# tjhladish/AbcSmc

Measured on AMD Instinct MI355X. Metric: particles/sec per SMC generation (PLS+weight+resample), 1/2/4/8 GPU, higher is better.
Workload: dtype f64 (inputs, model, distances, proposals, results; pair sums of the weight stage: fp64 operands as three f16 limbs on the matrix pipe + f32 v_exp_f32, weights <= 5e-7 rel of the fp64 oracle, largest seen 3.1e-7); 1 GPU; configs[2]: synthetic 1M particles x 16 params x 32 metrics, PLS 8 components, full generation; particles_per_gpu=1000000, particles_total=1000000, metrics=32, params=16, pls_components=8, pred_prior_size=100000, prev_pred_prior_size=100000, next_set_size=1000000, noise=MULTIVARIATE, ncomp_chosen=8, pls_component_rule=wilcoxon, parallelism=row-sharded x1, launcher=single GPU

## Files before the change

### abcsmc_amd/csrc/weights.hip

```cpp
#include <stdlib.h>

#include "abc_internal.h"
#include <hip/hip_ext.h>

namespace {

__device__ __forceinline__ double wave_sum(double v) {
#pragma unroll
    for (int o = 32; o >= 1; o >>= 1) v += __shfl_xor(v, o, 64);
    return v;
}

__device__ __forceinline__ double block_sum_256(double v, double* sm ) {
    v = wave_sum(v);
    __syncthreads();
    if ((threadIdx.x & 63) == 0) sm[threadIdx.x >> 6] = v;
    __syncthreads();
    return (sm[0] + sm[1]) + (sm[2] + sm[3]);
}

__global__ __launch_bounds__(256) void k_gather_rows(const double* __restrict__ Y, size_t n_local, size_t ldy,
                                                     int P, const unsigned long long* __restrict__ idx, size_t K,
                                                     unsigned long long idx_base, double* __restrict__ theta,
                                                     size_t ldt, const int* __restrict__ sel_fail, int* __restrict__ sel_fail_pin,
// ... 487 lines not shown
    double s = 0.0;
    for (int q = 0; q < n; q++) {
        const size_t j = sl[q];
        s += ks_pair_term<PP>(ai, ha, b + j * PP, hb[j]);
    }
    fix_j[i] = s;
}
template <int PP>
__global__ __launch_bounds__(256) void k_kde_fixups(const double* __restrict__ a, size_t kn, const double* __restrict__ b, size_t Kp,
                                                    const double* __restrict__ hb, const WConst* __restrict__ wc,
                                                    const unsigned char* __restrict__ far_flag, const unsigned* __restrict__ list,
                                                    unsigned nat, unsigned rb, unsigned slices, double* __restrict__ fix_i,
                                                    double* __restrict__ fix_j, const double* __restrict__ theta_raw, size_t K, size_t k0,
                                                    const double* __restrict__ prev_raw, double* __restrict__ part) {
    if (blockIdx.x < nat + rb) { far_body<PP>(blockIdx.x, a, kn, b, Kp, hb, wc, far_flag, list, nat, fix_i, fix_j); return; }
    const unsigned bid = blockIdx.x - (nat + rb);
    kde_body<PP>(bid % rb, bid / rb, slices, a, kn, b, Kp, hb, wc, theta_raw, K, k0, prev_raw, part, 1);
}

constexpr signed char KS_LA[KS_NP] = {0, 0, 1, 1, 2, 3};
constexpr signed char KS_LB[KS_NP] = {0, 1, 0, 1, 3, 2};
__device__ __forceinline__ float ks_max3(float a, float b, float c) {
    float r;
    asm volatile("v_max3_f32 %0, %1, %2, %3" : "=v"(r) : "v"(a), "v"(b), "v"(c));
    return r;
}
struct KsRef { float p0, p1, p2, p3; };
template <int V> __host__ __device__ constexpr int kz_nch() { return V > KS_TOPN ? V - KS_TOPN : V > KS_FOLD ? V - KS_FOLD : V; }
template <int V> __host__ __device__ constexpr bool kz_fold() { return V > KS_FOLD && V < KS_TOPN; }
template <int V> __host__ __device__ constexpr bool kz_topn() { return V > KS_TOPN; }
template <int V> __host__ __device__ constexpr int kz_nexact() { return V > KS_FOLD ? kz_nch<V>() : 1 + V; }
template <int NCH>
__host__ __device__ constexpr int kz_nsteps() { return kz_fold<NCH>() ? 1 + 6 * kz_nch<NCH>() : kz_topn<NCH>() ? 2 + 6 * kz_nch<NCH>() : 3 + 6 * NCH; }
template <int NCH, int S, typename AT>
__device__ __forceinline__ void kz_mfma(const AT A, const uint4* B, const uint4 (&NB)[2], const uint4& BN, f32x16& Z) {
    const f32x16 Z0 = {0.f, 0.f, 0.f, 0.f, 0.f, 0.f, 0.f, 0.f, 0.f, 0.f, 0.f, 0.f, 0.f, 0.f, 0.f, 0.f};
    if constexpr (kz_fold<NCH>()) {
        constexpr int C = kz_nch<NCH>();
        if constexpr (S == 0) {
            Z = __builtin_amdgcn_mfma_f32_32x32x16_f16(__builtin_bit_cast(f16x8, A[0]), __builtin_bit_cast(f16x8, B[0]), Z0, 0, 0, 0);
        } else if constexpr (S < C) {
            Z = __builtin_amdgcn_mfma_f32_32x32x16_f16(__builtin_bit_cast(f16x8, A[S * KS_NL]), __builtin_bit_cast(f16x8, B[S * KS_NL]), Z, 0, 0, 0);
        } else if constexpr (S == C) {
            Z = __builtin_amdgcn_mfma_f32_32x32x16_bf16(__builtin_bit_cast(bf16x8, NB[0]), __builtin_bit_cast(bf16x8, BN), Z, 0, 0, 0);
        } else {
            constexpr int q = S - (C + 1), c = q / 5, l = 1 + q % 5;
            Z = __builtin_amdgcn_mfma_f32_32x32x16_f16(__builtin_bit_cast(f16x8, A[c * KS_NL + KS_LA[l]]),
                                                       __builtin_bit_cast(f16x8, B[c * KS_NL + KS_LB[l]]), Z, 0, 0, 0);
        }
    } else if constexpr (kz_topn<NCH>()) {
        constexpr int C = kz_nch<NCH>();
        if constexpr (S == 0) {
            if (__builtin_amdgcn_readfirstlane(A[C * KS_NL + 1].y) == 0u) {
                Z = __builtin_amdgcn_mfma_f32_32x32x16_bf16(__builtin_bit_cast(bf16x8, A[C * KS_NL]), __builtin_bit_cast(bf16x8, NB[0]), Z0, 0, 0, 0);
                Z = __builtin_amdgcn_mfma_f32_32x32x16_f16(__builtin_bit_cast(f16x8, A[0]), __builtin_bit_cast(f16x8, B[0]), Z, 0, 0, 0);
            } else {
                Z = __builtin_amdgcn_mfma_f32_32x32x16_f16(__builtin_bit_cast(f16x8, A[0]), __builtin_bit_cast(f16x8, B[0]), Z0, 0, 0, 0);
            }
        } else if constexpr (S < C) {
            Z = __builtin_amdgcn_mfma_f32_32x32x16_f16(__builtin_bit_cast(f16x8, A[S * KS_NL]), __builtin_bit_cast(f16x8, B[S * KS_NL]), Z, 0, 0, 0);
        } else if constexpr (S == C) {
            Z = __builtin_amdgcn_mfma_f32_32x32x16_bf16(__builtin_bit_cast(bf16x8, A[C * KS_NL]), __builtin_bit_cast(bf16x8, BN), Z, 0, 0, 0);
        } else if constexpr (S == C + 1) {
            Z = __builtin_amdgcn_mfma_f32_32x32x16_bf16(__builtin_bit_cast(bf16x8, A[C * KS_NL]), __builtin_bit_cast(bf16x8, NB[1]), Z, 0, 0, 0);
        } else {
            constexpr int q = S - (C + 2), c = q / 5, l = 1 + q % 5;
            Z = __builtin_amdgcn_mfma_f32_32x32x16_f16(__builtin_bit_cast(f16x8, A[c * KS_NL + KS_LA[l]]),
                                                       __builtin_bit_cast(f16x8, B[c * KS_NL + KS_LB[l]]), Z, 0, 0, 0);
        }
    } else if constexpr (S == 0) {
        Z = __builtin_amdgcn_mfma_f32_32x32x16_bf16(__builtin_bit_cast(bf16x8, A[NCH * KS_NL]), __builtin_bit_cast(bf16x8, NB[0]), Z0, 0, 0, 0);
    } else if constexpr (S <= NCH) {
        constexpr int c = S - 1;
        Z = __builtin_amdgcn_mfma_f32_32x32x16_f16(__builtin_bit_cast(f16x8, A[c * KS_NL]), __builtin_bit_cast(f16x8, B[c * KS_NL]), Z, 0, 0, 0);
    } else if constexpr (S == NCH + 1) {
        Z = __builtin_amdgcn_mfma_f32_32x32x16_bf16(__builtin_bit_cast(bf16x8, A[NCH * KS_NL]), __builtin_bit_cast(bf16x8, BN), Z, 0, 0, 0);
    } else if constexpr (S == NCH + 2) {
        Z = __builtin_amdgcn_mfma_f32_32x32x16_bf16(__builtin_bit_cast(bf16x8, A[NCH * KS_NL]), __builtin_bit_cast(bf16x8, NB[1]), Z, 0, 0, 0);
    } else {
        constexpr int q = S - (NCH + 3), c = q / 5, l = 1 + q % 5;
        Z = __builtin_amdgcn_mfma_f32_32x32x16_f16(__builtin_bit_cast(f16x8, A[c * KS_NL + KS_LA[l]]),
                                                   __builtin_bit_cast(f16x8, B[c * KS_NL + KS_LB[l]]), Z, 0, 0, 0);
    }
}
template <int NCH, int S0, int S1, typename AT>
__device__ __forceinline__ void kz_mfma_range(const AT A, const uint4* B, const uint4 (&NB)[2], const uint4& BN, f32x16& Z) {
    if constexpr (S0 < S1) {
        kz_mfma<NCH, S0>(A, B, NB, BN, Z);
        kz_mfma_range<NCH, S0 + 1, S1>(A, B, NB, BN, Z);
    }
}
template <int V, typename AT>
__device__ __forceinline__ void kz_reference(const f32x16& Z, const AT A, const uint4& NB0, unsigned lane, int& n, uint4& BN) {
    const float f0 = __builtin_canonicalizef(Z[0]);
    __builtin_amdgcn_sched_barrier(0);
    const float m0 = ks_max3(f0, Z[1], Z[2]), m1 = ks_max3(Z[3], Z[4], Z[5]), m2 = ks_max3(Z[6], Z[7], Z[8]),
                m3 = ks_max3(Z[9], Z[10], Z[11]), m4 = ks_max3(Z[12], Z[13], Z[14]);
    const float ma = ks_max3(m0, m1, m2), mb = ks_max3(m3, m4, Z[15]);
    float m = ks_max3(ma, mb, mb);
    if constexpr (kz_topn<V>()) {
        const uint4 ti = A[kz_nch<V>() * KS_NL + 1];
        m -= __uint_as_float(ti.x);
        BN.x = NB0.x & ti.y;
        BN.y = NB0.y & ti.y;
    }
    const float nf = __builtin_floorf(m);
    n = (int)nf;
    typedef __attribute__((ext_vector_type(2))) float f32x2_;
    typedef __attribute__((ext_vector_type(2))) __bf16 bf16x2_;
    const bf16x2_ h1 = __builtin_convertvector((f32x2_){nf, 0.f}, bf16x2_);
    const float p1 = __uint_as_float(__builtin_bit_cast(unsigned, h1) << 16);
    const bf16x2_ pk = __builtin_convertvector((f32x2_){nf, nf - p1}, bf16x2_);
    (void)lane;
    BN.w = __builtin_bit_cast(unsigned, pk);
}
template <int NCH, int R, typename AT>
__device__ __forceinline__ void kz_slots(const AT An, const uint4* Bn, const uint4 (&NB)[2], f32x16& Zn, int& nn, unsigned lane,
                                         const f32x16& Zc, int nc, int hsub, double& s, KsRef& q, uint4& BN) {
    if constexpr (R < 8) {
        constexpr int NS = kz_nsteps<NCH>(), NA = kz_nexact<NCH>();
        if constexpr (R == 0) kz_mfma_range<NCH, 0, NA>(An, Bn, NB, BN, Zn);
        if constexpr (R == 3) {
            kz_reference<NCH>(Zn, An, NB[0], lane, nn, BN);
        }
        if constexpr (R >= 3 && R < 7) {
            constexpr int r = R - 3, M = NS - NA;
            constexpr int s0 = NA + (r * M) / 4, s1 = NA + ((r + 1) * M) / 4;
            if constexpr (r > 0) asm volatile("" : "+v"(Zn));
            kz_mfma_range<NCH, s0, s1>(An, Bn, NB, BN, Zn);
        }
#pragma unroll
        for (int g = 0; g < 2; g++) {
            const int i = R * 2 + g;
            const float e = __builtin_amdgcn_exp2f(Zc[i]);
            float& p = (i & 3) == 0 ? q.p0 : (i & 3) == 1 ? q.p1 : (i & 3) == 2 ? q.p2 : q.p3;
            if (i < 4) p = e; else p += e;
        }
        if constexpr (R == 7) {
            float t = q.p0 + q.p1;
            asm volatile("" : "+v"(t));
            t += q.p2 + q.p3;
            s += ldexp((double)t, nc - hsub);
            asm volatile("" : "+v"(s));
        } else {
            asm volatile("" : "+v"(q.p0), "+v"(q.p1), "+v"(q.p2), "+v"(q.p3));
        }
        __builtin_amdgcn_sched_barrier(0);
        kz_slots<NCH, R + 1>(An, Bn, NB, Zn, nn, lane, Zc, nc, hsub, s, q, BN);
    }
}

template <int NCH, int RO, int R, typename AT>
__device__ __forceinline__ void kz_fine(const AT An, const uint4* Bn, const uint4 (&NB)[2], f32x16& Zn, int& nn, unsigned lane,
                                        const f32x16& Zc, int nc, int hsub, double& s, KsRef& q, uint4& BN) {
    if constexpr (R < 16) {
        constexpr int NS = kz_nsteps<NCH>(), NA = kz_nexact<NCH>(), R0 = NA + RO, M = NS - NA, L = 16 - R0;
        if constexpr (R < NA) kz_mfma_range<NCH, R, R + 1>(An, Bn, NB, BN, Zn);
        if constexpr (R == R0) kz_reference<NCH>(Zn, An, NB[0], lane, nn, BN);
        if constexpr (R >= R0) {
            constexpr int r = R - R0;
            constexpr int s0 = NA + (r * M) / L, s1 = NA + ((r + 1) * M) / L;
            if constexpr (r > 0) asm volatile("" : "+v"(Zn));
            kz_mfma_range<NCH, s0, s1>(An, Bn, NB, BN, Zn);
        }
        {
            const float e = __builtin_amdgcn_exp2f(Zc[R]);
            float& p = (R & 3) == 0 ? q.p0 : (R & 3) == 1 ? q.p1 : (R & 3) == 2 ? q.p2 : q.p3;
            if (R < 4) p = e; else p += e;
        }
        if constexpr (R == 15) {
            float t = q.p0 + q.p1;
            asm volatile("" : "+v"(t));
            t += q.p2 + q.p3;
            s += ldexp((double)t, nc - hsub);
            asm volatile("" : "+v"(s));
        } else {
            asm volatile("" : "+v"(q.p0), "+v"(q.p1), "+v"(q.p2), "+v"(q.p3));
        }
        __builtin_amdgcn_sched_barrier(0);
        kz_fine<NCH, RO, R + 1>(An, Bn, NB, Zn, nn, lane, Zc, nc, hsub, s, q, BN);
    }
}
template <int NCH, int FINE, typename AT>
__device__ __forceinline__ void kz_step(const AT An, const uint4* Bn, const uint4 (&NB)[2], f32x16& Zn, int& nn, unsigned lane,
                                        const f32x16& Zc, int nc, int hsub, double& s, KsRef& q, uint4& BN) {
    if constexpr (FINE > 0) kz_fine<NCH, FINE, 0>(An, Bn, NB, Zn, nn, lane, Zc, nc, hsub, s, q, BN);
    else kz_slots<NCH, 0>(An, Bn, NB, Zn, nn, lane, Zc, nc, hsub, s, q, BN);
}

template <int NCH, int WPS, bool PING = (NCH >= 4), int FINE = 0>
__global__ __launch_bounds__(256, WPS) void k_kde_split(const uint4* __restrict__ at, size_t kn,
                                                      const uint4* __restrict__ bt, unsigned nbt,
                                                      const WConst* __restrict__ wc, const int* __restrict__ ha_int,
                                                      double* __restrict__ part, const uint2* __restrict__ tmin ) {
    if (!ks_split_on(wc)) return;
    constexpr int OPA = kz_nch<NCH>() * KS_NL, OPB = OPA + (kz_fold<NCH>() ? 0 : 1);
    constexpr int OPT = kz_topn<NCH>() ? 1 : 0;
    const unsigned lane = threadIdx.x & 63, wv = threadIdx.x >> 6;
    const size_t it0 = ((size_t)blockIdx.x * 4 + wv) * 2;
    const unsigned slices = gridDim.y, sl = blockIdx.y;
    const unsigned t0 = __builtin_amdgcn_readfirstlane((unsigned)((size_t)nbt * sl / slices));
    const unsigned t1 = __builtin_amdgcn_readfirstlane((unsigned)((size_t)nbt * (sl + 1) / slices));
    uint4 B0[OPA], B1[OPA];
#pragma unroll
    for (int q = 0; q < OPA; q++) {
        B0[q] = at[((it0 + 0) * OPA + q) * 64 + lane];
        B1[q] = at[((it0 + 1) * OPA + q) * 64 + lane];
    }
    uint4 NB[2];
    NB[0] = (lane < 32) ? make_uint4(KS_MONE | (KS_MONE << 16), KS_MONE, 0u, 0u) : make_uint4(0u, 0u, 0u, 0u);
    NB[1] = (lane < 32) ? make_uint4(0u, KS_MONE << 16, KS_MONE | (KS_MONE << 16), 0u) : make_uint4(0u, 0u, 0u, 0u);
    if constexpr (kz_fold<NCH>()) {
        const bool mine = (lane < 32) == (((lane & 31u) & 4u) == 0u);
        NB[0] = make_uint4(0u, 0u, 0u, mine ? (KS_MONE | (KS_MONE << 16)) : 0u);
    }
    const int hs0 = ha_int[(it0 + 0) * 32 + (lane & 31)], hs1 = ha_int[(it0 + 1) * 32 + (lane & 31)];
    double acc0 = 0.0, acc1 = 0.0;
    if (t0 < t1) {
        uint4 A[OPB + OPT];
#pragma unroll
        for (int q = 0; q < OPB; q++) A[q] = bt[((size_t)t0 * OPB + q) * 64 + lane];
        if constexpr (OPT) { const uint2 ti = tmin[t0]; A[OPB] = make_uint4(ti.x, ti.y, 0u, 0u); }
        f32x16 Z0, Z1;
        int n0 = 0, n1 = 0;
        uint4 BN = make_uint4(0u, 0u, 0u, 0u);
        {
            constexpr int NA = kz_nexact<NCH>();
            kz_mfma_range<NCH, 0, NA>(A, B0, NB, BN, Z0);
            kz_reference<NCH>(Z0, A, NB[0], lane, n0, BN);
            kz_mfma_range<NCH, NA, kz_nsteps<NCH>()>(A, B0, NB, BN, Z0);
        }
        if constexpr (!PING) {
        for (unsigned t = t0; t < t1; t++) {
            uint4 An[OPB + OPT];
            const unsigned tn = (t + 1 < t1) ? t + 1 : t;
#pragma unroll
            for (int q = 0; q < OPB; q++) An[q] = bt[((size_t)tn * OPB + q) * 64 + lane];
            if constexpr (OPT) { const uint2 ti = tmin[tn]; An[OPB] = make_uint4(ti.x, ti.y, 0u, 0u); }
            __builtin_amdgcn_sched_barrier(0);
            KsRef q;
            kz_step<NCH, FINE>(A, B1, NB, Z1, n1, lane, Z0, n0, hs0, acc0, q, BN);
            kz_step<NCH, FINE>(An, B0, NB, Z0, n0, lane, Z1, n1, hs1, acc1, q, BN);
#pragma unroll
            for (int q2 = 0; q2 < OPB; q2++) A[q2] = An[q2];
            if constexpr (OPT) { A[OPB].x = An[OPB].x; A[OPB].y = An[OPB].y; }
        }
        } else {
        uint4 An[OPB + OPT];
        for (unsigned t = t0; t < t1; t += 2) {
            {
                const unsigned tn = (t + 1 < t1) ? t + 1 : t;
#pragma unroll
                for (int q = 0; q < OPB; q++) An[q] = bt[((size_t)tn * OPB + q) * 64 + lane];
                if constexpr (OPT) { const uint2 ti = tmin[tn]; An[OPB] = make_uint4(ti.x, ti.y, 0u, 0u); }
            }
            __builtin_amdgcn_sched_barrier(0);
            KsRef q;
            kz_step<NCH, FINE>(A, B1, NB, Z1, n1, lane, Z0, n0, hs0, acc0, q, BN);
            kz_step<NCH, FINE>(An, B0, NB, Z0, n0, lane, Z1, n1, hs1, acc1, q, BN);
            if (t + 1 >= t1) break;
            {
                const unsigned tn = (t + 2 < t1) ? t + 2 : t + 1;
#pragma unroll
                for (int q2 = 0; q2 < OPB; q2++) A[q2] = bt[((size_t)tn * OPB + q2) * 64 + lane];
                if constexpr (OPT) { const uint2 ti = tmin[tn]; A[OPB] = make_uint4(ti.x, ti.y, 0u, 0u); }
            }
            __builtin_amdgcn_sched_barrier(0);
            kz_step<NCH, FINE>(An, B1, NB, Z1, n1, lane, Z0, n0, hs0, acc0, q, BN);
            kz_step<NCH, FINE>(A, B0, NB, Z0, n0, lane, Z1, n1, hs1, acc1, q, BN);
        }
        }
    }
    {
        const double v0 = acc0 + __shfl_xor(acc0, 32, 64);
        const double v1 = acc1 + __shfl_xor(acc1, 32, 64);
        const size_t i0 = (it0 + 0) * 32 + (lane & 31), i1 = (it0 + 1) * 32 + (lane & 31);
        if (lane < 32 && i0 < kn) part[(size_t)sl * kn + i0] = v0;
        if (lane < 32 && i1 < kn) part[(size_t)sl * kn + i1] = v1;
    }
}

template <int INFO>
struct KsLdsOps {
    const uint4* p;
    uint4 info;
    __device__ __forceinline__ const uint4& operator[](int i) const { return (INFO >= 0 && i == INFO) ? info : p[i * 64]; }
};
#ifndef KDE_LDS_F4
#define KDE_LDS_F4 0
#endif
#ifndef KDE_LDS_W3
#define KDE_LDS_W3 3
#endif
template <int NCH, int WPS, int FINE>
__global__ __launch_bounds__(256, WPS) void k_kde_split_lds(const uint4* __restrict__ at, size_t kn,
                                                          const uint4* __restrict__ bt, unsigned nbt,
                                                          const WConst* __restrict__ wc, const int* __restrict__ ha_int,
                                                          double* __restrict__ part, const uint2* __restrict__ tmin) {
    if (!ks_split_on(wc)) return;
    constexpr int OPA = kz_nch<NCH>() * KS_NL, OPB = OPA + (kz_fold<NCH>() ? 0 : 1);
    constexpr int OPT = kz_topn<NCH>() ? 1 : 0;
    constexpr int TILE = OPB * 64, NR = OPA / 4;
    __shared__ uint4 sA[2 * TILE];
    const unsigned lane = threadIdx.x & 63, wv = threadIdx.x >> 6;
    const size_t it0 = ((size_t)blockIdx.x * 4 + wv) * 2;
    const unsigned slices = gridDim.y, sl = blockIdx.y;
    const unsigned t0 = __builtin_amdgcn_readfirstlane((unsigned)((size_t)nbt * sl / slices));
    const unsigned t1 = __builtin_amdgcn_readfirstlane((unsigned)((size_t)nbt * (sl + 1) / slices));
    uint4 B0[OPA], B1[OPA];
#pragma unroll
    for (int q = 0; q < OPA; q++) {
        B0[q] = at[((it0 + 0) * OPA + q) * 64 + lane];
        B1[q] = at[((it0 + 1) * OPA + q) * 64 + lane];
    }
    uint4 NB[2];
    NB[0] = (lane < 32) ? make_uint4(KS_MONE | (KS_MONE << 16), KS_MONE, 0u, 0u) : make_uint4(0u, 0u, 0u, 0u);
    NB[1] = (lane < 32) ? make_uint4(0u, KS_MONE << 16, KS_MONE | (KS_MONE << 16), 0u) : make_uint4(0u, 0u, 0u, 0u);
    if constexpr (kz_fold<NCH>()) {
        const bool mine = (lane < 32) == (((lane & 31u) & 4u) == 0u);
        NB[0] = make_uint4(0u, 0u, 0u, mine ? (KS_MONE | (KS_MONE << 16)) : 0u);
    }
    const int hs0 = ha_int[(it0 + 0) * 32 + (lane & 31)], hs1 = ha_int[(it0 + 1) * 32 + (lane & 31)];
    double acc0 = 0.0, acc1 = 0.0;
    if (t0 < t1) {
        uint4 r[NR], r4 = make_uint4(0u, 0u, 0u, 0u);
        static_assert(OPA * 64 == NR * 256, "a tile's limb operands are whole rounds of the work-group");
#define KZ_TILE_FETCH(T)                                                                                            \
        {                                                                                                           \
            const uint4* src = bt + (size_t)(T) * (OPB * 64) + threadIdx.x;                                         \
            _Pragma("unroll") for (int j = 0; j < NR; j++) r[j] = src[256 * j];                                     \
            if constexpr (OPB > OPA) { if (threadIdx.x < 64) r4 = src[256 * NR]; }                                  \
        }
#define KZ_TILE_STORE(BUF)                                                                                          \
        {                                                                                                           \
            uint4* dst = sA + (BUF) * TILE + threadIdx.x;                                                           \
            _Pragma("unroll") for (int j = 0; j < NR; j++) dst[256 * j] = r[j];                                     \
            if constexpr (OPB > OPA) { if (threadIdx.x < 64) dst[256 * NR] = r4; }                                  \
        }
        KZ_TILE_FETCH(t0)
        KZ_TILE_STORE(0)
        __syncthreads();
        f32x16 Z0, Z1;
        int n0 = 0, n1 = 0;
        uint4 BN = make_uint4(0u, 0u, 0u, 0u);
        unsigned cur = 0;
        {
            constexpr int NA = kz_nexact<NCH>();
            KsLdsOps<OPT ? OPB : -1> A{sA + lane, make_uint4(0u, 0u, 0u, 0u)};
            if constexpr (OPT) { const uint2 ti = tmin[t0]; A.info = make_uint4(ti.x, ti.y, 0u, 0u); }
            kz_mfma_range<NCH, 0, NA>(A, B0, NB, BN, Z0);
            kz_reference<NCH>(Z0, A, NB[0], lane, n0, BN);
            kz_mfma_range<NCH, NA, kz_nsteps<NCH>()>(A, B0, NB, BN, Z0);
        }
        for (unsigned t = t0; t < t1; t++) {
            const unsigned tn = (t + 1 < t1) ? t + 1 : t;
            KZ_TILE_FETCH(tn)
            __builtin_amdgcn_sched_barrier(0);
            KsLdsOps<OPT ? OPB : -1> A{sA + cur * TILE + lane, make_uint4(0u, 0u, 0u, 0u)}, An{sA + (cur ^ 1u) * TILE + lane, make_uint4(0u, 0u, 0u, 0u)};
            if constexpr (OPT) {
                const uint2 ti = tmin[t], tj = tmin[tn];
                A.info = make_uint4(ti.x, ti.y, 0u, 0u);
                An.info = make_uint4(tj.x, tj.y, 0u, 0u);
            }
            KsRef q;
            kz_step<NCH, FINE>(A, B1, NB, Z1, n1, lane, Z0, n0, hs0, acc0, q, BN);
            KZ_TILE_STORE(cur ^ 1u)
            __syncthreads();
            kz_step<NCH, FINE>(An, B0, NB, Z0, n0, lane, Z1, n1, hs1, acc1, q, BN);
            cur ^= 1u;
        }
#undef KZ_TILE_FETCH
#undef KZ_TILE_STORE
    }
    {
        const double v0 = acc0 + __shfl_xor(acc0, 32, 64);
        const double v1 = acc1 + __shfl_xor(acc1, 32, 64);
        const size_t i0 = (it0 + 0) * 32 + (lane & 31), i1 = (it0 + 1) * 32 + (lane & 31);
        if (lane < 32 && i0 < kn) part[(size_t)sl * kn + i0] = v0;
        if (lane < 32 && i1 < kn) part[(size_t)sl * kn + i1] = v1;
    }
}

__device__ __forceinline__ double gaussian_pdf(double x, double sigma) {
    const double u = x / fabs(sigma);
    return (1.0 / (sqrt(2.0 * M_PI) * fabs(sigma))) * exp(-u * u / 2.0);
}

__device__ __forceinline__ double prior_likelihood(const abc_prior& pr, double v) {
    if (pr.kind == ABC_PRIOR_GAUSS) return gaussian_pdf(v - pr.a, pr.b);
    if (pr.kind == ABC_PRIOR_UNIF_INT)
        return ((v == round(v)) && (pr.a <= v) && (v <= pr.b)) ? 1.0 / (pr.b - pr.a + 1.0) : 0.0;
    return ((pr.a <= v) && (v <= pr.b)) ? 1.0 / (pr.b - pr.a) : 0.0;
}

constexpr unsigned SQ_INLINE_MAX = 4096;
__device__ __forceinline__ double sumsq_total(const double* __restrict__ sq_part, unsigned nparts, double* sm ) {
    double t = 0.0;
    for (unsigned j = threadIdx.x; j < nparts; j += 256) t += sq_part[j];
    return block_sum_256(t, sm);
}
__global__ __launch_bounds__(256) void k_sumsq_total(const double* __restrict__ sq_part, unsigned nparts, double* __restrict__ sq_total) {
    __shared__ double sm[4];
    const double t = sumsq_total(sq_part, nparts, sm);
    if (threadIdx.x == 0) *sq_total = t;
// ... 163 lines not shown
    for (int i = i0; i < i0 + per && i < total; i++) sum += bh[i];
    unsigned inc = sum;
#pragma unroll
    for (int o = 1; o < 64; o <<= 1) { const unsigned u = __shfl_up(inc, o, 64); if (lane >= o) inc += u; }
    if (lane == 63) wsum[wave] = inc;
    __syncthreads();
    unsigned run = inc - sum;
    for (int w = 0; w < wave; w++) run += wsum[w];
    for (int i = i0; i < i0 + per && i < total; i++) { const unsigned v = bh[i]; bh[i] = run; run += v; }
}
__global__ __launch_bounds__(256) void k_wq_rank(const double* __restrict__ hbk, size_t Kp, const WConst* __restrict__ wc,
                                                 const unsigned* __restrict__ bh, int nb, unsigned* __restrict__ rank) {
    __shared__ unsigned whist[4][256];
    __shared__ volatile unsigned woff[4][256];
    const int t = threadIdx.x, lane = t & 63, wave = t >> 6;
#pragma unroll
    for (int w = 0; w < 4; w++) whist[w][t] = 0;
    __syncthreads();
    const double lo = ks_okey_inv(wc->hb_lo), hi = ks_okey_inv(wc->hb_hi);
    const size_t seg = (size_t)blockIdx.x * WQ_CHUNK + (size_t)wave * (WQ_CHUNK / 4);
    unsigned q[WQ_ITEMS];
#pragma unroll
    for (int j = 0; j < WQ_ITEMS; j++) {
        const size_t i = seg + (size_t)j * 64 + lane;
        q[j] = (i < Kp) ? ks_qbin(hbk[i], lo, hi) : 0u;
        if (i < Kp) atomicAdd(&whist[wave][q[j]], 1u);
    }
    __syncthreads();
    {
        unsigned run = bh[(size_t)t * nb + blockIdx.x];
#pragma unroll
        for (int w = 0; w < 4; w++) { woff[w][t] = run; run += whist[w][t]; }
    }
    __syncthreads();
    const unsigned long long lt_mask = (lane == 0) ? 0ull : (~0ull >> (64 - lane));
#pragma unroll
    for (int j = 0; j < WQ_ITEMS; j++) {
        const size_t i = seg + (size_t)j * 64 + lane;
        const bool valid = i < Kp;
        const unsigned d = q[j];
        unsigned long long peers = __ballot(valid);
#pragma unroll
        for (int b = 0; b < 8; b++) {
            const unsigned long long m = __ballot((d >> b) & 1u);
            peers &= ((d >> b) & 1u) ? m : ~m;
        }
        if (valid) rank[i] = woff[wave][d] + (unsigned)__popcll(peers & lt_mask);
        __builtin_amdgcn_wave_barrier();
        if (valid && (peers & lt_mask) == 0) woff[wave][d] += (unsigned)__popcll(peers);
        __builtin_amdgcn_wave_barrier();
    }
}
constexpr float KS_TOPN_SPREAD = 0.75f;
__global__ __launch_bounds__(256) void k_tile_tmin(const float* __restrict__ topf, size_t ntiles, uint2* __restrict__ tinfo) {
    const size_t t = (size_t)blockIdx.x * 256 + threadIdx.x;
    if (t >= ntiles) return;
    float mn = 3.0e38f, mx = -3.0e38f;
    for (int j = 0; j < 32; j++) {
        const float v = topf[t * 32 + j];
        if (v < (float)KS_HB_ZERO) { mn = v < mn ? v : mn; mx = v > mx ? v : mx; }
    }
    if (mx < mn) { mn = (float)KS_HB_ZERO; mx = mn; }
    const bool wide = !(mx - mn <= KS_TOPN_SPREAD);
    tinfo[t] = wide ? make_uint2(0u, 0u) : make_uint2(__float_as_uint(mn), 0xffffffffu);
}
static double ks_topn_min_pairs() {
    const char* e = abc_diag_env("ABC_KDE_TOPN_MIN_PAIRS");
    const double minp = e ? atof(e) : 4.0e9;
    return minp;
}

using WrowsFn = decltype(&k_wrows<1>);
struct WrowsEntry { WrowsFn fn; int div; };
static const WrowsEntry WROWS[4] = {{k_wrows<1>, 32}, {k_wrows<2>, 16}, {k_wrows<4, 3>, 8}, {k_wrows<4>, 8}};

using SplitFn = decltype(&k_kde_split<1, 3, true, 1>);
static const SplitFn KDE_SPLIT[3][4] = {
    {k_kde_split<1, 3, true, 1>,
     k_kde_split<2, 2>,
     k_kde_split_lds<3, KDE_LDS_W3, KDE_LDS_F4>,
     k_kde_split_lds<4, 2, KDE_LDS_F4>},
    {k_kde_split<KS_FOLD + 1, 3, true, 1>,
     k_kde_split<KS_FOLD + 2, 2, false, 0>,
     k_kde_split_lds<KS_FOLD + 3, KDE_LDS_W3, KDE_LDS_F4>,
     k_kde_split_lds<KS_FOLD + 4, 2, KDE_LDS_F4>},
    {k_kde_split<KS_TOPN + 1, 3, true, 1>,
     k_kde_split<KS_TOPN + 2, 2, false, 0>,
     k_kde_split_lds<KS_TOPN + 3, KDE_LDS_W3, KDE_LDS_F4>,
     k_kde_split_lds<KS_TOPN + 4, 2, KDE_LDS_F4>},
};

using KdeFn = decltype(&k_kde<2>);
using EpanFn = decltype(&k_epan<2>);
using FixupsFn = decltype(&k_kde_fixups<8>);
static const KdeFn KDE_FP64[7] = {nullptr, k_kde<2>, k_kde<4>, k_kde<8>, k_kde<16>, k_kde<32>, k_kde<64>};
static const EpanFn KDE_EPAN[7] = {nullptr, k_epan<2>, k_epan<4>, k_epan<8>, k_epan<16>, k_epan<32>, k_epan<64>};
static const FixupsFn KDE_FIXUPS[7] = {nullptr, nullptr, nullptr, k_kde_fixups<8>, k_kde_fixups<16>, k_kde_fixups<32>, k_kde_fixups<64>};
static int ks_lg(int PP) { return __builtin_ctz((unsigned)PP); }

static void launch_wrows(const abc_wplan& pl, hipStream_t s, int is_prev, const double* in, size_t rows, size_t ld, size_t P, WConst* wc,
                         const double* w, double* out, double* hb, unsigned short* tiles, unsigned char* far_flag, unsigned* far_list,
                         int* ha_int, double* ha_frac, const unsigned* rank, float* topf) {
    const WrowsEntry& e = WROWS[pl.NCH - 1];
    const size_t rows_pad = (is_prev ? pl.nbt : pl.nat) * 32;
    hipLaunchKernelGGL(e.fn, dim3((unsigned)((rows_pad / e.div + 3) / 4)), dim3(256), 0, s, in, rows, ld, (int)P, pl.PP, rows_pad, wc,
                       w, is_prev, out, hb, tiles, is_prev ? pl.opb : pl.opa, far_flag, far_list, ha_int, ha_frac, pl.fold ? 1 : 0, rank, topf);
}

int launch_weights_prev(abc_ctx* ctx, size_t P, size_t kn_max, const double* theta_prev, size_t Kp, const double* w_prev,
                        const double* dv_prev, abc_wprev* out, hipStream_t st) {
    memset(out, 0, sizeof(*out));
    if (P > (size_t)W_MAXP) ABC_FAIL(ctx, ABC_ERR_UNSUPPORTED, "weights: P = %zu > %d parameters", P, W_MAXP);
    if (Kp > 0xffffffffull) ABC_FAIL(ctx, ABC_ERR_UNSUPPORTED, "weights: K' = %zu >= 2^32", Kp);
    hipStream_t s = st ? st : ctx->stream;
    const abc_wplan pl = abc_weights_plan(P, kn_max, Kp, ctx->kde_mode, ctx->weight_kernel, ks_topn_min_pairs());
    const int PP = pl.PP;
    const bool split = pl.split, topn = pl.topn;
    const size_t nbt = pl.nbt;
    WConst* wc = (WConst*)abc_ws_alloc(ctx, sizeof(WConst));
    double* b = (double*)abc_ws_alloc(ctx, Kp * PP * sizeof(double));
    double* hb = (double*)abc_ws_alloc(ctx, Kp * sizeof(double));
    double* cpart = (double*)abc_ws_alloc(ctx, (P > 64 ? P : 64) * WC_NB * sizeof(double));
    unsigned short* bt = nullptr;
    unsigned* far_list = nullptr;
    unsigned* rank = nullptr;
    uint2* tmin = nullptr;
    float* topf = nullptr;
    double* hbk = nullptr;
    unsigned* qh = nullptr;
    if (split) {
        bt = (unsigned short*)abc_ws_alloc(ctx, nbt * pl.opb * 1024);
        far_list = (unsigned*)abc_ws_alloc(ctx, KS_MAX_FAR_J * sizeof(unsigned));
        if (!bt || !far_list) ABC_FAIL(ctx, ABC_ERR_NOMEM, "weights: workspace exhausted");
        if (topn) {
            rank = (unsigned*)abc_ws_alloc(ctx, Kp * sizeof(unsigned));
            tmin = (uint2*)abc_ws_alloc(ctx, nbt * sizeof(uint2));
            topf = (float*)abc_ws_alloc(ctx, nbt * 32 * sizeof(float));
            hbk = (double*)abc_ws_alloc(ctx, Kp * sizeof(double));
            qh = (unsigned*)abc_ws_alloc(ctx, (size_t)256 * ((Kp + WQ_CHUNK - 1) / WQ_CHUNK) * sizeof(unsigned));
            if (!rank || !tmin || !topf || !hbk || !qh) ABC_FAIL(ctx, ABC_ERR_NOMEM, "weights: workspace exhausted");
        }
    }
    if (!wc || !b || !hb || !cpart) ABC_FAIL(ctx, ABC_ERR_NOMEM, "weights: workspace exhausted");
    const double* centre = (const double*)((const char*)wc + offsetof(WConst, centre));
    hipLaunchKernelGGL(k_wprep, dim3(1), dim3(64), 0, s, dv_prev, (int)P, wc, pl.lim_i);
    hipLaunchKernelGGL(k_wcentre, dim3((unsigned)P, WC_NB), dim3(256), 0, s, theta_prev, Kp, wc, cpart);
    hipLaunchKernelGGL(k_wcentre_finish, dim3(1), dim3(P > 64 ? 1024 : 64), 0, s, theta_prev, Kp, (int)P, cpart, wc);
    if (topn) {
        const int nbq = (int)((Kp + WQ_CHUNK - 1) / WQ_CHUNK);
        hipLaunchKernelGGL(k_whb, dim3((unsigned)((Kp + 255) / 256)), dim3(256), 0, s, theta_prev, Kp, (int)P, wc, w_prev, hbk);
        hipLaunchKernelGGL(k_wq_hist, dim3(nbq), dim3(256), 0, s, (const double*)hbk, Kp, (const WConst*)wc, qh, nbq);
        hipLaunchKernelGGL(k_wq_scan, dim3(1), dim3(1024), 0, s, qh, 256 * nbq);
        hipLaunchKernelGGL(k_wq_rank, dim3(nbq), dim3(256), 0, s, (const double*)hbk, Kp, (const WConst*)wc, (const unsigned*)qh, nbq, rank);
        ABC_HIP(ctx, hipGetLastError());
    }
    if (split) {
        launch_wrows(pl, s, 1, theta_prev, Kp, Kp, P, wc, w_prev, b, hb, bt, nullptr, far_list, nullptr, nullptr, rank, topf);
    } else {
        hipLaunchKernelGGL(k_wscale, dim3((unsigned)((Kp + 255) / 256)), dim3(256), 0, s, theta_prev, Kp, Kp,
                           (int)P, PP, wc, centre, (size_t)1, w_prev, b, hb);
    }
    if (topn) hipLaunchKernelGGL(k_tile_tmin, dim3((unsigned)((nbt + 255) / 256)), dim3(256), 0, s, (const float*)topf, nbt, tmin);
    ABC_HIP(ctx, hipGetLastError());
    out->wc = wc; out->b = b; out->hb = hb; out->bt = bt; out->far_list = far_list; out->tmin = (unsigned*)tmin;
    out->Kp = Kp; out->P = P; out->kn_max = kn_max; out->split = split ? 1 : 0; out->ready = 1;
    return ABC_OK;
}

int launch_weights_raw(abc_ctx* ctx, const abc_prior* priors, const double* theta, size_t K, size_t P, size_t k0,
                       size_t kn, const double* theta_prev, size_t Kp, const double* w_prev, const double* dv_prev,
                       double* w_raw, const abc_wprev* prev, const double** sumsq_out) {
    if (sumsq_out) *sumsq_out = nullptr;
    if (P > (size_t)W_MAXP) ABC_FAIL(ctx, ABC_ERR_UNSUPPORTED, "weights: P = %zu > %d parameters", P, W_MAXP);
    if (kn == 0) return ABC_OK;
    ABC_TRY(abc_kde_words(ctx));
    if (Kp > 0xffffffffull) ABC_FAIL(ctx, ABC_ERR_UNSUPPORTED, "weights: K' = %zu >= 2^32", Kp);
    if (k0 + kn > K) ABC_FAIL(ctx, ABC_ERR_INVALID, "weights: row range [%zu,%zu) outside K=%zu", k0, k0 + kn, K);
    abc_wplan pl = abc_weights_plan(P, kn, Kp, ctx->kde_mode, ctx->weight_kernel, ks_topn_min_pairs());
    const int PP = pl.PP;
    const bool epan = pl.epan, split = pl.split;
    const size_t rb = pl.rb, slices = pl.slices, nbt = pl.nbt, nat = pl.nat;
    abc_wprev own;
    if (!prev || !prev->ready) {
        ABC_TRY(launch_weights_prev(ctx, P, kn, theta_prev, Kp, w_prev, dv_prev, &own, nullptr));
        prev = &own;
    }
    if (prev->Kp != Kp || prev->P != P || prev->kn_max < kn || (prev->split != 0) != split)
        ABC_FAIL(ctx, ABC_ERR_INVALID, "weights: the prepared previous set does not match this call");
    abc_weights_plan_topn(&pl, prev->tmin != nullptr);
    WConst* wc = (WConst*)prev->wc;
    double* b = prev->b;
    double* hb = prev->hb;
    unsigned short* bt = prev->bt;
    unsigned* far_list = prev->far_list;
    double* a = (double*)abc_ws_alloc(ctx, kn * PP * sizeof(double));
    double* part = (double*)abc_ws_alloc(ctx, slices * kn * sizeof(double));
    unsigned short* at = nullptr;
    unsigned char* far_flag = nullptr;
    double *fix_i = nullptr, *fix_j = nullptr, *ha_frac = nullptr;
    int* ha_int = nullptr;
    if (split) {
        at = (unsigned short*)abc_ws_alloc(ctx, nat * pl.opa * 1024);
        far_flag = (unsigned char*)abc_ws_alloc(ctx, nat * 32);
        fix_i = (double*)abc_ws_alloc(ctx, kn * sizeof(double));
        fix_j = (double*)abc_ws_alloc(ctx, kn * sizeof(double));
        ha_frac = (double*)abc_ws_alloc(ctx, nat * 32 * sizeof(double));
        ha_int = (int*)abc_ws_alloc(ctx, nat * 32 * sizeof(int));
        if (!at || !far_flag || !fix_i || !fix_j || !ha_frac || !ha_int) ABC_FAIL(ctx, ABC_ERR_NOMEM, "weights: workspace exhausted");
    }
    if (!a || !part) ABC_FAIL(ctx, ABC_ERR_NOMEM, "weights: workspace exhausted");
    const double* centre = (const double*)((const char*)wc + offsetof(WConst, centre));
    StageTimer tm(ctx, ST_WEIGHTS_MISC);
    if (split) {
        launch_wrows(pl, ctx->stream, 0, theta + k0, kn, K, P, wc, nullptr, a, nullptr, at, far_flag, far_list, ha_int, ha_frac, nullptr, nullptr);
    } else {
// ... 74 lines not shown
```

Baseline: 372.9 million particles/s.

## Add two-tile interleaved pair-sum path for single-chunk fold/topn KDE split kernels

Adds a new kz_pair_sums path, selected via a TPB=2 template parameter, for the one-chunk fold and topn variants of the split KDE kernel. It processes two B tiles per step with interleaved MFMA chains and a joint max reference, and prefetches the next A tiles inside the step pipeline so loads and exp2 work overlap the matrix ops. Supporting changes pre-shuffle the wide-tile bias operand in k_tile_tmin, seed the BN operand at init, and use a perm-based bf16 split of the reference exponent. The aim is better MFMA/VALU overlap and fewer reference computations per tile. The cost is much more register pressure, a different reduction order, and more complex tail handling.

```diff
diff --git a/abcsmc_amd/csrc/weights.hip b/abcsmc_amd/csrc/weights.hip
--- a/abcsmc_amd/csrc/weights.hip
+++ b/abcsmc_amd/csrc/weights.hip
@@ -563,7 +563,9 @@
         constexpr int C = kz_nch<NCH>();
         if constexpr (S == 0) {
             if (__builtin_amdgcn_readfirstlane(A[C * KS_NL + 1].y) == 0u) {
-                Z = __builtin_amdgcn_mfma_f32_32x32x16_bf16(__builtin_bit_cast(bf16x8, A[C * KS_NL]), __builtin_bit_cast(bf16x8, NB[0]), Z0, 0, 0, 0);
+                const bool hi = __builtin_amdgcn_mbcnt_hi(~0u, __builtin_amdgcn_mbcnt_lo(~0u, 0u)) >= 32u;
+                const uint4 NT = make_uint4(hi ? (KS_MONE | (KS_MONE << 16)) : 0u, hi ? KS_MONE : 0u, 0u, 0u);
+                Z = __builtin_amdgcn_mfma_f32_32x32x16_bf16(__builtin_bit_cast(bf16x8, A[C * KS_NL]), __builtin_bit_cast(bf16x8, NT), Z0, 0, 0, 0);
                 Z = __builtin_amdgcn_mfma_f32_32x32x16_f16(__builtin_bit_cast(f16x8, A[0]), __builtin_bit_cast(f16x8, B[0]), Z, 0, 0, 0);
             } else {
                 Z = __builtin_amdgcn_mfma_f32_32x32x16_f16(__builtin_bit_cast(f16x8, A[0]), __builtin_bit_cast(f16x8, B[0]), Z0, 0, 0, 0);
@@ -594,6 +596,10 @@
                                                    __builtin_bit_cast(f16x8, B[c * KS_NL + KS_LB[l]]), Z, 0, 0, 0);
     }
 }
+template <int V>
+__device__ __forceinline__ uint4 kz_bn_init(const uint4& NB0) {
+    return kz_topn<V>() ? make_uint4(NB0.x, NB0.y, 0u, 0u) : make_uint4(0u, 0u, 0u, 0u);
+}
 template <int NCH, int S0, int S1, typename AT>
 __device__ __forceinline__ void kz_mfma_range(const AT A, const uint4* B, const uint4 (&NB)[2], const uint4& BN, f32x16& Z) {
     if constexpr (S0 < S1) {
@@ -601,29 +607,27 @@
         kz_mfma_range<NCH, S0 + 1, S1>(A, B, NB, BN, Z);
     }
 }
-template <int V, typename AT>
-__device__ __forceinline__ void kz_reference(const f32x16& Z, const AT A, const uint4& NB0, unsigned lane, int& n, uint4& BN) {
+__device__ __forceinline__ void kz_nsplit(float m, int& n, uint4& BN) {
+    const float nf = __builtin_floorf(m);
+    n = (int)nf;
+    const unsigned nb = __float_as_uint(nf);
+    const float p2 = nf - __uint_as_float(nb & 0xffff0000u);
+    BN.w = __builtin_amdgcn_perm(__float_as_uint(p2), nb, 0x07060302u);
+}
+__device__ __forceinline__ float kz_max16(const f32x16& Z) {
     const float f0 = __builtin_canonicalizef(Z[0]);
     __builtin_amdgcn_sched_barrier(0);
     const float m0 = ks_max3(f0, Z[1], Z[2]), m1 = ks_max3(Z[3], Z[4], Z[5]), m2 = ks_max3(Z[6], Z[7], Z[8]),
                 m3 = ks_max3(Z[9], Z[10], Z[11]), m4 = ks_max3(Z[12], Z[13], Z[14]);
     const float ma = ks_max3(m0, m1, m2), mb = ks_max3(m3, m4, Z[15]);
-    float m = ks_max3(ma, mb, mb);
-    if constexpr (kz_topn<V>()) {
-        const uint4 ti = A[kz_nch<V>() * KS_NL + 1];
-        m -= __uint_as_float(ti.x);
-        BN.x = NB0.x & ti.y;
-        BN.y = NB0.y & ti.y;
-    }
-    const float nf = __builtin_floorf(m);
-    n = (int)nf;
-    typedef __attribute__((ext_vector_type(2))) float f32x2_;
-    typedef __attribute__((ext_vector_type(2))) __bf16 bf16x2_;
-    const bf16x2_ h1 = __builtin_convertvector((f32x2_){nf, 0.f}, bf16x2_);
-    const float p1 = __uint_as_float(__builtin_bit_cast(unsigned, h1) << 16);
-    const bf16x2_ pk = __builtin_convertvector((f32x2_){nf, nf - p1}, bf16x2_);
+    return ks_max3(ma, mb, mb);
+}
+template <int V, typename AT>
+__device__ __forceinline__ void kz_reference(const f32x16& Z, const AT A, unsigned lane, int& n, uint4& BN) {
+    float m = kz_max16(Z);
+    if constexpr (kz_topn<V>()) m -= __uint_as_float(A[kz_nch<V>() * KS_NL + 1].x);
     (void)lane;
-    BN.w = __builtin_bit_cast(unsigned, pk);
+    kz_nsplit(m, n, BN);
 }
 template <int NCH, int R, typename AT>
 __device__ __forceinline__ void kz_slots(const AT An, const uint4* Bn, const uint4 (&NB)[2], f32x16& Zn, int& nn, unsigned lane,
@@ -632,7 +636,7 @@
         constexpr int NS = kz_nsteps<NCH>(), NA = kz_nexact<NCH>();
         if constexpr (R == 0) kz_mfma_range<NCH, 0, NA>(An, Bn, NB, BN, Zn);
         if constexpr (R == 3) {
-            kz_reference<NCH>(Zn, An, NB[0], lane, nn, BN);
+            kz_reference<NCH>(Zn, An, lane, nn, BN);
         }
         if constexpr (R >= 3 && R < 7) {
             constexpr int r = R - 3, M = NS - NA;
@@ -667,7 +671,7 @@
     if constexpr (R < 16) {
         constexpr int NS = kz_nsteps<NCH>(), NA = kz_nexact<NCH>(), R0 = NA + RO, M = NS - NA, L = 16 - R0;
         if constexpr (R < NA) kz_mfma_range<NCH, R, R + 1>(An, Bn, NB, BN, Zn);
-        if constexpr (R == R0) kz_reference<NCH>(Zn, An, NB[0], lane, nn, BN);
+        if constexpr (R == R0) kz_reference<NCH>(Zn, An, lane, nn, BN);
         if constexpr (R >= R0) {
             constexpr int r = R - R0;
             constexpr int s0 = NA + (r * M) / L, s1 = NA + ((r + 1) * M) / L;
@@ -699,12 +703,19 @@
     else kz_slots<NCH, 0>(An, Bn, NB, Zn, nn, lane, Zc, nc, hsub, s, q, BN);
 }
 
-template <int NCH, int WPS, bool PING = (NCH >= 4), int FINE = 0>
+template <int V>
+__device__ __forceinline__ void kz_pair_sums(const uint4* __restrict__ at, size_t kn, const uint4* __restrict__ bt, unsigned nbt,
+                                             const int* __restrict__ ha_int, double* __restrict__ part, const uint2* __restrict__ tmin);
+template <int NCH, int WPS, bool PING = (NCH >= 4), int FINE = 0, int TPB = 1>
 __global__ __launch_bounds__(256, WPS) void k_kde_split(const uint4* __restrict__ at, size_t kn,
                                                       const uint4* __restrict__ bt, unsigned nbt,
                                                       const WConst* __restrict__ wc, const int* __restrict__ ha_int,
                                                       double* __restrict__ part, const uint2* __restrict__ tmin ) {
     if (!ks_split_on(wc)) return;
+    if constexpr (TPB == 2) {
+        kz_pair_sums<NCH>(at, kn, bt, nbt, ha_int, part, tmin);
+        return;
+    }
     constexpr int OPA = kz_nch<NCH>() * KS_NL, OPB = OPA + (kz_fold<NCH>() ? 0 : 1);
     constexpr int OPT = kz_topn<NCH>() ? 1 : 0;
     const unsigned lane = threadIdx.x & 63, wv = threadIdx.x >> 6;
@@ -734,11 +745,11 @@
         if constexpr (OPT) { const uint2 ti = tmin[t0]; A[OPB] = make_uint4(ti.x, ti.y, 0u, 0u); }
         f32x16 Z0, Z1;
         int n0 = 0, n1 = 0;
-        uint4 BN = make_uint4(0u, 0u, 0u, 0u);
+        uint4 BN = kz_bn_init<NCH>(NB[0]);
         {
             constexpr int NA = kz_nexact<NCH>();
             kz_mfma_range<NCH, 0, NA>(A, B0, NB, BN, Z0);
-            kz_reference<NCH>(Z0, A, NB[0], lane, n0, BN);
+            kz_reference<NCH>(Z0, A, lane, n0, BN);
             kz_mfma_range<NCH, NA, kz_nsteps<NCH>()>(A, B0, NB, BN, Z0);
         }
         if constexpr (!PING) {
@@ -785,6 +796,194 @@
     {
         const double v0 = acc0 + __shfl_xor(acc0, 32, 64);
         const double v1 = acc1 + __shfl_xor(acc1, 32, 64);
+        const size_t i0 = (it0 + 0) * 32 + (lane & 31), i1 = (it0 + 1) * 32 + (lane & 31);
+        if (lane < 32 && i0 < kn) part[(size_t)sl * kn + i0] = v0;
+        if (lane < 32 && i1 < kn) part[(size_t)sl * kn + i1] = v1;
+    }
+}
+
+template <int V, int J0, int J1>
+__device__ __forceinline__ void kz_rest(const uint4* A0, const uint4* A1, const uint4* B, const uint4 (&NB)[2], const uint4& BN,
+                                        f32x16& Z0, f32x16& Z1) {
+    if constexpr (J0 < J1) {
+        constexpr int NA = kz_nexact<V>(), H = kz_nsteps<V>() - NA;
+        if constexpr (J0 < H) {
+            asm volatile("" : "+v"(Z0));
+            kz_mfma<V, NA + J0>(A0, B, NB, BN, Z0);
+        } else {
+            asm volatile("" : "+v"(Z1));
+            kz_mfma<V, NA + J0 - H>(A1, B, NB, BN, Z1);
+        }
+        kz_rest<V, J0 + 1, J1>(A0, A1, B, NB, BN, Z0, Z1);
+    }
+}
+template <int V>
+__device__ __forceinline__ void kz_reference2(const f32x16& Z0, const f32x16& Z1, const uint4* A0, const uint4* A1, int& n, uint4& BN) {
+    float m;
+    if constexpr (kz_topn<V>()) {
+        constexpr int I = kz_nch<V>() * KS_NL + 1;
+        const float ma = kz_max16(Z0) - __uint_as_float(A0[I].x), mb = kz_max16(Z1) - __uint_as_float(A1[I].x);
+        m = ks_max3(ma, mb, mb);
+    } else {
+        const float f0 = __builtin_canonicalizef(Z0[0]), g0 = __builtin_canonicalizef(Z1[0]);
+        __builtin_amdgcn_sched_barrier(0);
+        const float a0 = ks_max3(f0, Z0[1], Z0[2]), a1 = ks_max3(Z0[3], Z0[4], Z0[5]), a2 = ks_max3(Z0[6], Z0[7], Z0[8]),
+                    a3 = ks_max3(Z0[9], Z0[10], Z0[11]), a4 = ks_max3(Z0[12], Z0[13], Z0[14]);
+        const float b0 = ks_max3(g0, Z1[1], Z1[2]), b1 = ks_max3(Z1[3], Z1[4], Z1[5]), b2 = ks_max3(Z1[6], Z1[7], Z1[8]),
+                    b3 = ks_max3(Z1[9], Z1[10], Z1[11]), b4 = ks_max3(Z1[12], Z1[13], Z1[14]);
+        const float c0 = ks_max3(a0, a1, a2), c1 = ks_max3(a3, a4, Z0[15]), c2 = ks_max3(b0, b1, b2), c3 = ks_max3(b3, b4, Z1[15]);
+        const float d = ks_max3(c0, c1, c2);
+        m = ks_max3(d, c3, c3);
+    }
+    kz_nsplit(m, n, BN);
+}
+template <int V, int MT>
+__device__ __forceinline__ void kz_chain(const uint4* A0, const uint4* A1, const uint4* B, const uint4 (&NB)[2], uint4& BN,
+                                         f32x16& Z0, f32x16& Z1, int& n, unsigned lane) {
+    constexpr int NA = kz_nexact<V>(), H = kz_nsteps<V>() - NA;
+    kz_mfma_range<V, 0, NA>(A0, B, NB, BN, Z0);
+    if constexpr (MT == 2) {
+        kz_mfma_range<V, 0, NA>(A1, B, NB, BN, Z1);
+        kz_reference2<V>(Z0, Z1, A0, A1, n, BN);
+    } else {
+        kz_reference<V>(Z0, A0, lane, n, BN);
+    }
+    kz_rest<V, 0, MT * H>(A0, A1, B, NB, BN, Z0, Z1);
+}
+template <int V, int MT, int VT, bool LD, int R, int NOP>
+__device__ __forceinline__ void kz_pstep(uint4 (&A0)[NOP], uint4 (&A1)[NOP], const uint4* Bn, const uint4 (&NB)[2], f32x16& Zn0,
+                                         f32x16& Zn1, int& nn, unsigned lane, const f32x16& Zc0, const f32x16& Zc1, int nc,
+                                         double& s, float (&p)[8], uint4& BN, const uint4* nx0, const uint4* nx1, const uint2* ni0,
+                                         const uint2* ni1) {
+    constexpr int SL = 16 * VT;
+    if constexpr (R < SL) {
+        constexpr int NA = kz_nexact<V>(), H = kz_nsteps<V>() - NA, E = MT * NA, R0 = E + 1, M = MT * H, L = SL - R0;
+        constexpr int OPN = NOP - (kz_topn<V>() ? 1 : 0);
+        if constexpr (R < E) {
+            if constexpr (R < NA) kz_mfma<V, R>(A0, Bn, NB, BN, Zn0);
+            else kz_mfma<V, R - NA>(A1, Bn, NB, BN, Zn1);
+        }
+        if constexpr (MT == 2 && R == R0) kz_reference2<V>(Zn0, Zn1, A0, A1, nn, BN);
+        if constexpr (MT == 1 && R == R0) kz_reference<V>(Zn0, A0, lane, nn, BN);
+        if constexpr (MT > 0 && R >= R0) {
+            constexpr int r = R - R0, j0 = (r * M) / L, j1 = ((r + 1) * M) / L;
+            kz_rest<V, j0, j1>(A0, A1, Bn, NB, BN, Zn0, Zn1);
+            if constexpr (LD && j0 < H && j1 >= H) {
+#pragma unroll
+                for (int q = 0; q < OPN; q++) A0[q] = nx0[q * 64 + lane];
+                if constexpr (kz_topn<V>()) { const uint2 ti = *ni0; A0[OPN] = make_uint4(ti.x, ti.y, 0u, 0u); }
+            }
+            if constexpr (LD && R == SL - 1) {
+#pragma unroll
+                for (int q = 0; q < OPN; q++) A1[q] = nx1[q * 64 + lane];
+                if constexpr (kz_topn<V>()) { const uint2 ti = *ni1; A1[OPN] = make_uint4(ti.x, ti.y, 0u, 0u); }
+            }
+        }
+        {
+            const float e = __builtin_amdgcn_exp2f(R < 16 ? Zc0[R & 15] : Zc1[R & 15]);
+            constexpr int c = (R & 3) + (R < 16 ? 0 : 4);
+            if constexpr ((R & 15) < 4) p[c] = e; else p[c] += e;
+        }
+        if constexpr (R == SL - 1) {
+            float t = p[0] + p[1];
+            asm volatile("" : "+v"(t));
+            t += p[2] + p[3];
+            if constexpr (VT == 2) {
+                float u = p[4] + p[5];
+                asm volatile("" : "+v"(u));
+                u += p[6] + p[7];
+                asm volatile("" : "+v"(t), "+v"(u));
+                t += u;
+            }
+            s += ldexp((double)t, nc);
+            asm volatile("" : "+v"(s));
+        } else if constexpr (R < 16) {
+            asm volatile("" : "+v"(p[0]), "+v"(p[1]), "+v"(p[2]), "+v"(p[3]));
+        } else {
+            asm volatile("" : "+v"(p[0]), "+v"(p[1]), "+v"(p[2]), "+v"(p[3]), "+v"(p[4]), "+v"(p[5]), "+v"(p[6]), "+v"(p[7]));
+        }
+        __builtin_amdgcn_sched_barrier(0);
+        kz_pstep<V, MT, VT, LD, R + 1>(A0, A1, Bn, NB, Zn0, Zn1, nn, lane, Zc0, Zc1, nc, s, p, BN, nx0, nx1, ni0, ni1);
+    }
+}
+
+template <int V>
+__device__ __forceinline__ void kz_pair_sums(const uint4* __restrict__ at, size_t kn, const uint4* __restrict__ bt, unsigned nbt,
+                                             const int* __restrict__ ha_int, double* __restrict__ part, const uint2* __restrict__ tmin) {
+    static_assert(kz_nch<V>() == 1, "one chunk");
+    constexpr int OPA = KS_NL, OPB = OPA + (kz_fold<V>() ? 0 : 1);
+    constexpr int OPT = kz_topn<V>() ? 1 : 0;
+    constexpr size_t TS = (size_t)OPB * 64;
+    const unsigned lane = threadIdx.x & 63, wv = __builtin_amdgcn_readfirstlane(threadIdx.x >> 6);
+    const size_t it0 = ((size_t)blockIdx.x * 4 + wv) * 2;
+    const unsigned slices = gridDim.y, sl = blockIdx.y;
+    const unsigned t0 = __builtin_amdgcn_readfirstlane((unsigned)((size_t)nbt * sl / slices));
+    const unsigned t1 = __builtin_amdgcn_readfirstlane((unsigned)((size_t)nbt * (sl + 1) / slices));
+    uint4 B0[OPA], B1[OPA];
+#pragma unroll
+    for (int q = 0; q < OPA; q++) {
+        B0[q] = at[((it0 + 0) * OPA + q) * 64 + lane];
+        B1[q] = at[((it0 + 1) * OPA + q) * 64 + lane];
+    }
+    uint4 NB[2];
+    NB[0] = (lane < 32) ? make_uint4(KS_MONE | (KS_MONE << 16), KS_MONE, 0u, 0u) : make_uint4(0u, 0u, 0u, 0u);
+    NB[1] = (lane < 32) ? make_uint4(0u, KS_MONE << 16, KS_MONE | (KS_MONE << 16), 0u) : make_uint4(0u, 0u, 0u, 0u);
+    uint4 BN = kz_bn_init<V>(NB[0]);
+    if constexpr (kz_fold<V>()) {
+        const bool mine = (lane < 32) == (((lane & 31u) & 4u) == 0u);
+        NB[0] = make_uint4(0u, 0u, 0u, mine ? (KS_MONE | (KS_MONE << 16)) : 0u);
+    }
+    double acc0 = 0.0, acc1 = 0.0;
+    if (t0 < t1) {
+        const unsigned np = (t1 - t0) >> 1;
+        const bool odd = ((t1 - t0) & 1u) != 0u;
+        const uint4* tb = bt + (size_t)t0 * TS;
+        const uint2* ib = OPT ? tmin + t0 : tmin;
+        uint4 A0[OPB + OPT], A1[OPB + OPT];
+        f32x16 Za0, Za1, Zb0, Zb1;
+        int na = 0, nb = 0;
+        float p[8];
+#pragma unroll
+        for (int q = 0; q < OPB; q++) A0[q] = tb[q * 64 + lane];
+        if constexpr (OPT) { const uint2 ti = ib[0]; A0[OPB] = make_uint4(ti.x, ti.y, 0u, 0u); }
+        if (np > 0) {
+#pragma unroll
+            for (int q = 0; q < OPB; q++) A1[q] = tb[TS + q * 64 + lane];
+            if constexpr (OPT) { const uint2 ti = ib[1]; A1[OPB] = make_uint4(ti.x, ti.y, 0u, 0u); }
+            kz_chain<V, 2>(A0, A1, B0, NB, BN, Za0, Za1, na, lane);
+        } else {
+            kz_chain<V, 1>(A0, A1, B0, NB, BN, Za0, Za1, na, lane);
+        }
+        for (unsigned k = 1; k < np; k++) {
+            const uint4 *nx0 = tb + 2 * TS, *nx1 = tb + 3 * TS;
+            const uint2 *ni0 = ib + (OPT ? 2 : 0), *ni1 = ib + (OPT ? 3 : 0);
+            __builtin_amdgcn_sched_barrier(0);
+            kz_pstep<V, 2, 2, true, 0>(A0, A1, B1, NB, Zb0, Zb1, nb, lane, Za0, Za1, na, acc0, p, BN, nx0, nx1, ni0, ni1);
+            kz_pstep<V, 2, 2, false, 0>(A0, A1, B0, NB, Za0, Za1, na, lane, Zb0, Zb1, nb, acc1, p, BN, nx0, nx1, ni0, ni1);
+            tb = nx0;
+            ib = ni0;
+        }
+        if (np > 0) {
+            const uint4* nx0 = tb + (odd ? 2 * TS : 0);
+            const uint2* ni0 = ib + ((OPT && odd) ? 2 : 0);
+            kz_pstep<V, 2, 2, true, 0>(A0, A1, B1, NB, Zb0, Zb1, nb, lane, Za0, Za1, na, acc0, p, BN, nx0, tb, ni0, ib);
+            if (odd) {
+                kz_pstep<V, 1, 2, false, 0>(A0, A1, B0, NB, Za0, Za1, na, lane, Zb0, Zb1, nb, acc1, p, BN, nx0, tb, ni0, ib);
+            } else {
+                kz_pstep<V, 0, 2, false, 0>(A0, A1, B0, NB, Za0, Za1, na, lane, Zb0, Zb1, nb, acc1, p, BN, nx0, tb, ni0, ib);
+            }
+            tb = nx0;
+            ib = ni0;
+        }
+        if (odd) {
+            kz_pstep<V, 1, 1, false, 0>(A0, A1, B1, NB, Zb0, Zb1, nb, lane, Za0, Za1, na, acc0, p, BN, tb, tb, ib, ib);
+            kz_pstep<V, 0, 1, false, 0>(A0, A1, B0, NB, Za0, Za1, na, lane, Zb0, Zb1, nb, acc1, p, BN, tb, tb, ib, ib);
+        }
+    }
+    {
+        const int hs0 = ha_int[(it0 + 0) * 32 + (lane & 31)], hs1 = ha_int[(it0 + 1) * 32 + (lane & 31)];
+        const double v0 = ldexp(acc0 + __shfl_xor(acc0, 32, 64), -hs0);
+        const double v1 = ldexp(acc1 + __shfl_xor(acc1, 32, 64), -hs1);
         const size_t i0 = (it0 + 0) * 32 + (lane & 31), i1 = (it0 + 1) * 32 + (lane & 31);
         if (lane < 32 && i0 < kn) part[(size_t)sl * kn + i0] = v0;
         if (lane < 32 && i1 < kn) part[(size_t)sl * kn + i1] = v1;
@@ -853,14 +1052,14 @@
         __syncthreads();
         f32x16 Z0, Z1;
         int n0 = 0, n1 = 0;
-        uint4 BN = make_uint4(0u, 0u, 0u, 0u);
+        uint4 BN = kz_bn_init<NCH>(NB[0]);
         unsigned cur = 0;
         {
             constexpr int NA = kz_nexact<NCH>();
             KsLdsOps<OPT ? OPB : -1> A{sA + lane, make_uint4(0u, 0u, 0u, 0u)};
             if constexpr (OPT) { const uint2 ti = tmin[t0]; A.info = make_uint4(ti.x, ti.y, 0u, 0u); }
             kz_mfma_range<NCH, 0, NA>(A, B0, NB, BN, Z0);
-            kz_reference<NCH>(Z0, A, NB[0], lane, n0, BN);
+            kz_reference<NCH>(Z0, A, lane, n0, BN);
             kz_mfma_range<NCH, NA, kz_nsteps<NCH>()>(A, B0, NB, BN, Z0);
         }
         for (unsigned t = t0; t < t1; t++) {
@@ -1130,7 +1329,8 @@
     }
 }
 constexpr float KS_TOPN_SPREAD = 0.75f;
-__global__ __launch_bounds__(256) void k_tile_tmin(const float* __restrict__ topf, size_t ntiles, uint2* __restrict__ tinfo) {
+__global__ __launch_bounds__(256) void k_tile_tmin(const float* __restrict__ topf, size_t ntiles, uint2* __restrict__ tinfo,
+                                                   unsigned short* __restrict__ tiles, int ops) {
     const size_t t = (size_t)blockIdx.x * 256 + threadIdx.x;
     if (t >= ntiles) return;
     float mn = 3.0e38f, mx = -3.0e38f;
@@ -1141,6 +1341,18 @@
     if (mx < mn) { mn = (float)KS_HB_ZERO; mx = mn; }
     const bool wide = !(mx - mn <= KS_TOPN_SPREAD);
     tinfo[t] = wide ? make_uint2(0u, 0u) : make_uint2(__float_as_uint(mn), 0xffffffffu);
+    if (wide) {
+        uint4* ob = (uint4*)(tiles + (t * (size_t)ops + (size_t)(ops - 1)) * 512);
+        for (int j = 0; j < 32; j++) {
+            uint4 lo = ob[j], hi = ob[32 + j];
+            hi.x = lo.x;
+            hi.y = lo.y & 0xffffu;
+            lo.x = 0u;
+            lo.y &= 0xffff0000u;
+            ob[j] = lo;
+            ob[32 + j] = hi;
+        }
+    }
 }
 static double ks_topn_min_pairs() {
     const char* e = abc_diag_env("ABC_KDE_TOPN_MIN_PAIRS");
@@ -1158,11 +1370,11 @@
      k_kde_split<2, 2>,
      k_kde_split_lds<3, KDE_LDS_W3, KDE_LDS_F4>,
      k_kde_split_lds<4, 2, KDE_LDS_F4>},
-    {k_kde_split<KS_FOLD + 1, 3, true, 1>,
+    {k_kde_split<KS_FOLD + 1, 3, true, 1, 2>,
      k_kde_split<KS_FOLD + 2, 2, false, 0>,
      k_kde_split_lds<KS_FOLD + 3, KDE_LDS_W3, KDE_LDS_F4>,
      k_kde_split_lds<KS_FOLD + 4, 2, KDE_LDS_F4>},
-    {k_kde_split<KS_TOPN + 1, 3, true, 1>,
+    {k_kde_split<KS_TOPN + 1, 3, true, 1, 2>,
      k_kde_split<KS_TOPN + 2, 2, false, 0>,
      k_kde_split_lds<KS_TOPN + 3, KDE_LDS_W3, KDE_LDS_F4>,
      k_kde_split_lds<KS_TOPN + 4, 2, KDE_LDS_F4>},
@@ -1238,7 +1450,7 @@
         hipLaunchKernelGGL(k_wscale, dim3((unsigned)((Kp + 255) / 256)), dim3(256), 0, s, theta_prev, Kp, Kp,
                            (int)P, PP, wc, centre, (size_t)1, w_prev, b, hb);
     }
-    if (topn) hipLaunchKernelGGL(k_tile_tmin, dim3((unsigned)((nbt + 255) / 256)), dim3(256), 0, s, (const float*)topf, nbt, tmin);
+    if (topn) hipLaunchKernelGGL(k_tile_tmin, dim3((unsigned)((nbt + 255) / 256)), dim3(256), 0, s, (const float*)topf, nbt, tmin, bt, pl.opb);
     ABC_HIP(ctx, hipGetLastError());
     out->wc = wc; out->b = b; out->hb = hb; out->bt = bt; out->far_list = far_list; out->tmin = (unsigned*)tmin;
     out->Kp = Kp; out->P = P; out->kn_max = kn_max; out->split = split ? 1 : 0; out->ready = 1;
```

New measurement: 383.1 million particles/s, median of 6. 1.03x the previous value.
